# MystenLabs/dapol

Measured on AMD Instinct MI355X. Metric: entities/sec (tree build + 64-bit range-proof gen), 2^20 leaves, 1/2/4/8 GPU, higher is better.
Workload: dtype int32 limbs (255-bit modular integers)

## Files before the change

### dapol_amd/csrc/host_range.inc

```

#include <cstdlib>
#include "policy_plan.inc"
#include "prove_plan.inc"

struct MsmTiming {
    std::vector<hipEvent_t> ev;
    std::vector<int> kind;
    size_t used = 0;
    bool enabled = false;
    size_t kernels[2] = {0, 0};
    ~MsmTiming() { for (auto e : ev) (void)hipEventDestroy(e); }
    hipError_t mark(hipStream_t st, int k = 0) {
        if (!enabled) return hipSuccess;
        if (used == ev.size()) {
            hipEvent_t e;
            hipError_t r = hipEventCreate(&e);
            if (r != hipSuccess) return r;
            ev.push_back(e);
        }
        if ((used & 1) == 0) { if (kind.size() <= used / 2) kind.push_back(k); else kind[used / 2] = k; }
        return hipEventRecord(ev[used++], st);
    }
    void count(int k, size_t n) { if (enabled) kernels[k] += n; }
    double total_ms(int k) {
// ... 192 lines not shown
}

static int32_t queue_chunk(dapol_ctx* ctx, const ProvePlan& P, const ProveLane& L, RangeArgs A, hipStream_t st, ForkGuard& fg, uint32_t* d_err,
                           MsmTiming* tm) {
    const size_t cb = A.B;
    const int fs_shape = P.fs_shape, nf_rounds = P.nf_rounds();
    sc* const stab_buf = A.stab;
    if (!P.stab_main) A.stab = nullptr;
    const unsigned g_wave = (unsigned)cb, g_lane = nblk(cb, 64), g_dig = (unsigned)(cb * (size_t)(A.TP / 64));
    const unsigned g_gsdig = nblk(cb * (size_t)(2 * A.N), 64);
    hipLaunchKernelGGL(k_rp_nonce_key, dim3(g_lane), dim3(64), 0, st, A); LAUNCH_CHECK();
    if (P.gs) hipLaunchKernelGGL(k_rp_nonces_gs, dim3(g_gsdig), dim3(64), 0, st, A);
    else hipLaunchKernelGGL(k_rp_nonces, dim3(g_dig), dim3(64), 0, st, A);
    LAUNCH_CHECK();
    if (P.side_A) {
        HIPCHK(hipEventRecord(ctx->ev_fork, st));
        HIPCHK(hipStreamWaitEvent(ctx->side[2], ctx->ev_fork, 0));
        fg.forked(2);
        hipLaunchKernelGGL(k_rp_A, dim3(g_wave), dim3(64), 0, ctx->side[2], A, ctx->tv); LAUNCH_CHECK();
        HIPCHK(hipEventRecord(ctx->ev_join[2], ctx->side[2]));
        FAULT_AFTER_FORK("prove_A");
    } else if (P.a_lane(cb)) {
        hipLaunchKernelGGL(k_rp_A_lane, dim3(g_lane), dim3(64), 0, st, A, ctx->tv); LAUNCH_CHECK();
    } else {
        hipLaunchKernelGGL(k_rp_A, dim3(g_wave), dim3(64), 0, st, A, ctx->tv); LAUNCH_CHECK();
    }
    if (tm) HIPCHK(tm->mark(st));
    launch_main_msm(ctx, P, L, A, st, -1, tm); LAUNCH_CHECK();
    if (tm) HIPCHK(tm->mark(st));
    if (P.side_A) { HIPCHK(hipStreamWaitEvent(st, ctx->ev_join[2], 0)); fg.joined(2); }
    LAUNCH_FS(k_rp_finish1, fs_shape, cb, st, A, ctx->tv); LAUNCH_CHECK();
    hipLaunchKernelGGL(k_rp_poly, dim3(g_wave * (unsigned)A.fs_parts), dim3(64), 0, st, A); LAUNCH_CHECK();
    LAUNCH_FS(k_rp_finish2, fs_shape, cb, st, A, ctx->tv); LAUNCH_CHECK();
    hipLaunchKernelGGL(k_rp_lr, dim3(g_wave * (unsigned)A.fs_parts), dim3(64), 0, st, A); LAUNCH_CHECK();
    if (fs_shape == 2) hipLaunchKernelGGL(k_rp_finish3<2>, dim3(g_wave), dim3(64), 0, st, A);
    else hipLaunchKernelGGL(k_rp_finish3<0>, dim3(g_lane), dim3(64), 0, st, A);
    LAUNCH_CHECK();
    for (int k = 0; k < nf_rounds; k++) {
        if (P.gs) hipLaunchKernelGGL(k_rp_round_prep_gs, dim3(g_gsdig), dim3(64), 0, st, A, k);
        else hipLaunchKernelGGL(k_rp_round_prep, dim3(g_dig), dim3(64), 0, st, A, k);
        LAUNCH_CHECK();
        hipLaunchKernelGGL(k_rp_round_ip, dim3(g_wave), dim3(64), 0, st, A, k); LAUNCH_CHECK();
        if (tm) HIPCHK(tm->mark(st));
        launch_main_msm(ctx, P, L, A, st, k, tm); LAUNCH_CHECK();
        if (tm) HIPCHK(tm->mark(st));
        LAUNCH_FS(k_rp_round_finish, fs_shape, cb, st, A, ctx->tv, k); LAUNCH_CHECK();
        hipLaunchKernelGGL(k_rp_fold, dim3(fold_blocks(A, cb, k)), dim3(256), 0, st, A, k);
        LAUNCH_CHECK();
    }
    if (nf_rounds == A.lgN) {
        hipLaunchKernelGGL(k_rp_final, dim3(g_lane), dim3(64), 0, st, A, d_err); LAUNCH_CHECK();
        return DAPOL_OK;
    }
    if (P.gs_mat) hipLaunchKernelGGL(k_rp_mat_prep_gs, dim3(g_gsdig), dim3(64), 0, st, A);
    else hipLaunchKernelGGL(k_rp_mat_prep, dim3(g_dig), dim3(64), 0, st, A);
    LAUNCH_CHECK();
    if (tm) HIPCHK(tm->mark(st, 1));
    { int32_t rc = launch_materialise(ctx, P, L, A, st, tm); if (rc) return rc; }
    if (tm) HIPCHK(tm->mark(st, 1));
    const unsigned g_tail = (unsigned)(cb * (size_t)(P.tail_n / 32));
    {
        RangeArgs Ai = A;
        Ai.stab = P.stab_tail ? stab_buf : nullptr;
        if (P.tail_rpl == 4) hipLaunchKernelGGL(k_rp_tail_table4, dim3(nblk(cb * (size_t)(2 * P.tail_n / 4), 64)), dim3(64), 0, st, Ai);
        else hipLaunchKernelGGL(k_rp_tail_table, dim3(g_tail), dim3(64), 0, st, Ai);
        LAUNCH_CHECK();
    }
    RangeArgs At = A;
    At.N = P.tail_n; At.lgN = P.tail_lgn; At.TP = 2 * P.tail_n; At.wbits = TAIL_WBITS; At.nwin = TAIL_NWIN; At.nsplit = 0;
    At.a = A.tail_a; At.b = A.tail_b; At.s1 = A.tail_s1; At.s2 = A.tail_s2;
    At.stab = P.stab_tail ? stab_buf : nullptr;
    At.out_round0 = nf_rounds;
    const TableView tvt{A.tailT, 1, TAIL_WBITS, 0, 0};
    for (int k = 0; k < P.tail_lgn; k++) {
        hipLaunchKernelGGL(k_rp_round_prep, dim3(g_tail), dim3(64), 0, st, At, k); LAUNCH_CHECK();
        hipLaunchKernelGGL(k_rp_round_ip, dim3(g_wave), dim3(64), 0, st, At, k); LAUNCH_CHECK();
        if (P.tail_gs) {
            hipLaunchKernelGGL(k_rp_tail_gs, dim3(nblk(2 * cb, TAIL_GS_LISTS)), dim3(TAIL_GS_BLOCK), 0, st, At, tvt, k, L.gsacc); LAUNCH_CHECK();
            hipLaunchKernelGGL(k_rp_tail_combine, dim3(nblk(2 * cb, 64)), dim3(64), 0, st, At, L.gsacc);
        } else launch_msm_tail(st, At, tvt, k, P.tail_lpl);
        LAUNCH_CHECK();
        LAUNCH_FS(k_rp_round_finish, fs_shape, cb, st, At, ctx->tv, k); LAUNCH_CHECK();
        hipLaunchKernelGGL(k_rp_fold, dim3(fold_blocks(At, cb, k)), dim3(256), 0, st, At, k);
        LAUNCH_CHECK();
    }
    hipLaunchKernelGGL(k_rp_final, dim3(g_lane), dim3(64), 0, st, At, d_err); LAUNCH_CHECK();
    return DAPOL_OK;
}

static int32_t range_prove_device(dapol_ctx* ctx, int n, int m, size_t B, const uint64_t* d_vals, const uint32_t* d_blind,
                                  const uint32_t* d_Vc, const uint32_t* d_seed, const uint64_t* d_stream, uint64_t slot_base,
                                  const uint32_t* d_tape, uint32_t* d_out, MsmTiming* tm, size_t tape_stride = 0, uint32_t sub_k = 1,
                                  size_t out_stride = 0, PendingProve* pend = nullptr) {
    ProveShape s{};
    s.n = n; s.m = m; s.B = B;
    s.tail_length = ctx->opt.tail_length; s.small_call_max = ctx->opt.small_call_max; s.generator_stationary = ctx->opt.generator_stationary;
    s.streams = ctx->opt.streams; s.gs_tile_rows = ctx->opt.gs_tile_rows; s.gs_slices = ctx->opt.gs_slices; s.chunk_proofs = ctx->opt.chunk_proofs;
    s.wbits = ctx->tv.wbits; s.nwin = ctx->tv.nwin_c(); s.hi_split = ctx->tv.hi_split;
    s.n_cu = ctx->n_cu; s.resident_waves = ctx->resident_waves();
    s.budget_bytes = scratch_budget_bytes(ctx);
    s.timed = tm != nullptr;
    ProvePlan P = plan_range_prove(s);
    for (bool lowered = false;; lowered = true) {
        hipError_t e = ctx->scratch.ensure(P.lane_bytes() * P.nlanes);
        if (e == hipSuccess) {
            if (lowered) P.finalise(s, P.chunk, P.nlanes);
            break;
        }
        (void)hipGetLastError();
        if (e != hipErrorOutOfMemory || (P.nlanes == 1 && P.chunk <= 64)) return fail_hip(e, "scratch allocation", __FILE__, __LINE__);
        if (P.nlanes > 1) P.nlanes--;
        else P.chunk = (P.chunk + 1) / 2;
    }
    const size_t chunk = P.chunk, slots = (size_t)m * (2 * (size_t)n + 4);
    const int nlanes = P.nlanes;
    RangeArgs A{};
    A.n = n; A.m = m; A.N = P.N; A.lgN = P.lgN; A.TP = P.TP;
    A.out_words = 72 + 16 * A.lgN;
    A.seed = d_seed; A.slot_base = slot_base;
    A.wbits = s.wbits; A.nwin = s.nwin;
    A.tail_n = P.tail_n; A.use_hi = P.use_hi ? 1 : 0; A.fs_parts = P.fs_parts; A.mat_round = P.nf_rounds();
    A.stream_id = d_stream;
    A.tape_stride = (uint32_t)(tape_stride ? tape_stride : slots);
    A.tape = d_tape;
    A.sub_k = sub_k ? sub_k : 1; A.sub_slots = (uint32_t)slots;
    A.out = d_out; A.out_stride = out_stride ? out_stride : (size_t)A.out_words;
    ProveLane lanes[4];
    hipStream_t lane_stream[4] = {ctx->stream, ctx->side[0], ctx->side[1], ctx->side[2]};
    for (int ln = 0; ln < nlanes; ln++) lanes[ln] = carve_lane(P, A, (uint8_t*)ctx->scratch.p + P.lane_bytes() * ln);
    DevBuf<uint32_t> err_own;
    DevBuf<uint32_t>& err = pend ? pend->err : err_own;
    HIPCHK(err.alloc(1));
    HIPCHK(hipMemsetAsync(err.p, 0, 4, ctx->stream));
    ForkGuard fg(ctx);
    if (nlanes > 1) {
        HIPCHK(hipEventRecord(ctx->ev_fork, ctx->stream));
        for (int ln = 1; ln < nlanes; ln++) { HIPCHK(hipStreamWaitEvent(lane_stream[ln], ctx->ev_fork, 0)); fg.forked(ln - 1); }
    }
    size_t chunk_no = 0;
    for (size_t first = 0; first < B; first += chunk, chunk_no++) {
        const int ln = (int)(chunk_no % (size_t)nlanes);
        if (chunk_no == 2) FAULT_AFTER_FORK("prove_lanes");
        RangeArgs Ac = lanes[ln].A;
        Ac.B = B - first < chunk ? B - first : chunk;
        Ac.vals = d_vals + first * m;
        Ac.blind = d_blind + first * m * 8;
        Ac.Vc = d_Vc + first * m * 8;
        Ac.p0 = first;
        int32_t rc = queue_chunk(ctx, P, lanes[ln], Ac, lane_stream[ln], fg, err.p, tm);
        if (rc) return rc;
    }
    for (int ln = 1; ln < nlanes; ln++) {
        HIPCHK(hipEventRecord(ctx->ev_join[ln - 1], lane_stream[ln]));
        HIPCHK(hipStreamWaitEvent(ctx->stream, ctx->ev_join[ln - 1], 0));
        fg.joined(ln - 1);
    }
    if (pend) {
        pend->ctx = ctx;
        pend->h_err_p = ctx->h_pinned + pend->pinned_slot;
        HIPCHK(hipMemcpyAsync(pend->h_err_p, err.p, 4, hipMemcpyDeviceToHost, ctx->stream));
        pend->armed = true;
        return DAPOL_OK;
    }
    uint32_t h_err = 0;
    HIPCHK(hipMemcpyAsync(&h_err, err.p, 4, hipMemcpyDeviceToHost, ctx->stream));
    HIPCHK(hipStreamSynchronize(ctx->stream));
    if (h_err) return fail(DAPOL_ERR_INVALID_ARGUMENT, "prover drew a zero challenge (ProofError::MaliciousDealer)");
    return DAPOL_OK;
}

struct EventPair {
    hipEvent_t a = nullptr, b = nullptr;
    ~EventPair() { if (a) (void)hipEventDestroy(a); if (b) (void)hipEventDestroy(b); }
// ... 43 lines not shown
```

### dapol_amd/csrc/kernels_range.h

```cpp
#pragma once
#include <hip/hip_runtime.h>
#include <type_traits>
#include "kernels_ctx_tree.h"
#include "ge_quad.h"

namespace dapol {

struct ProofState {
    uint64_t strobe[25];
    uint32_t pos, pos_begin;
    uint32_t err, pad_;
    sc y, z, y_inv, x, w, u, u_inv;
    sc a_bl, s_bl, t1, t2, t1_bl, t2_bl, t_x, cL, cR;
    uint32_t nkey[8];
};

struct RangeArgs {
    int n, m, N, lgN, TP;
    int wbits, nwin;
    size_t B;
    const uint64_t* vals;
    const uint32_t* blind;
    const uint32_t* Vc;
    const uint32_t* seed;
    const uint64_t* stream_id;
    uint64_t slot_base;
    const uint32_t* tape;
    uint32_t tape_stride;
    uint32_t sub_k, sub_slots;
    size_t p0;
    sc* a; sc* b; sc* s1; sc* s2;
    sc* stab;
    dig_t* dig;
    int nsplit;
    int use_hi;
    int fs_parts;
    sc* fs_part;
    ProofState* st;
    int32_t* PA; int32_t* P0; int32_t* P1;
    int mat_round;
    int tail_n;
    int32_t* tailT;
    sc* tail_a; sc* tail_b; sc* tail_s1; sc* tail_s2;
    uint32_t* out;
    size_t out_stride;
    int out_words;
    int out_round0;
};

#ifndef DAPOL_TAIL_WBITS
#define DAPOL_TAIL_WBITS 5
#endif
enum { TAIL_WBITS = DAPOL_TAIL_WBITS, TAIL_NWIN = 253 / TAIL_WBITS + 1, TAIL_ENTRIES = (1 << (TAIL_WBITS - 1)) + 1, TAIL_ROW_WORDS = TAIL_ENTRIES * 32 };
enum { MSM_PLAIN = 0, MSM_MATERIALIZE = 1, MSM_TAIL = 2 };
enum { STAB_ROUNDS = 6, STAB_N = 1 << STAB_ROUNDS };

__device__ __forceinline__ void proof_row(const RangeArgs& A, size_t b, size_t& e, uint32_t& j) {
    const size_t g = A.p0 + b;
    if (A.sub_k <= 1) { e = g; j = 0; }
    else { e = g / A.sub_k; j = (uint32_t)(g - e * A.sub_k); }
}
__device__ __forceinline__ uint32_t* proof_out(const RangeArgs& A, size_t b) {
    size_t e; uint32_t j;
    proof_row(A, b, e, j);
    return A.out + e * A.out_stride + (size_t)j * (size_t)A.out_words;
}
__device__ __forceinline__ void tape_wide(uint32_t* w16, const RangeArgs& A, size_t b, uint32_t slot) {
    size_t e; uint32_t j;
    proof_row(A, b, e, j);
    const uint32_t first = j * A.sub_slots;
    if (A.tape) {
        const uint4* p = reinterpret_cast<const uint4*>(A.tape + (e * (size_t)A.tape_stride + first + slot) * 16);
        for (int i = 0; i < 4; i++) { uint4 q = p[i]; w16[4 * i] = q.x; w16[4 * i + 1] = q.y; w16[4 * i + 2] = q.z; w16[4 * i + 3] = q.w; }
    } else {
        uint32_t key[8];
        for (int i = 0; i < 8; i++) key[i] = A.st[b].nkey[i];
        seed_wide(w16, key, 2u, A.stream_id[e], A.slot_base + first + slot);
    }
}
__global__ __launch_bounds__(64) void k_rp_nonce_key(RangeArgs A) {
    size_t b = (size_t)blockIdx.x * 64 + threadIdx.x;
    if (b >= A.B || A.tape) return;
    uint32_t key[8], w[16];
    for (int i = 0; i < 8; i++) key[i] = A.seed[i];
    size_t e; uint32_t sj;
    proof_row(A, b, e, sj);
    seed_wide(w, key, 6u, A.stream_id[e], A.slot_base + (uint64_t)sj * A.sub_slots);
    for (int i = 0; i < 8; i++) key[i] = w[i];
    seed_wide(w, key, 7u, (uint64_t)A.n, (uint64_t)A.m);
    for (int i = 0; i < 8; i++) key[i] = w[i];
    for (int j0 = 0; j0 < A.m; j0 += 31) {
        const int n_ent = 1 + ((A.m - j0 < 31) ? A.m - j0 : 31);
        const int n_blk = (n_ent + 1) / 2;
        uint32_t cv[8], blk[16], o[16];
        blake3_iv(cv);
        for (int i = 0; i < n_blk; i++) {
            for (int h = 0; h < 2; h++) {
                const int e = 2 * i + h;
                if (e == 0) { for (int k = 0; k < 8; k++) blk[k] = key[k]; }
                else if (e < n_ent) ld8(blk + 8 * h, A.Vc + (b * A.m + j0 + e - 1) * 8);
                else { for (int k = 0; k < 8; k++) blk[8 + k] = 0; }
            }
            const bool last = i == n_blk - 1;
            blake3_compress(o, cv, blk, 0, (last && (n_ent & 1)) ? 32u : 64u, (i == 0 ? B3_CHUNK_START : 0u) | (last ? (B3_CHUNK_END | B3_ROOT) : 0u));
            for (int k = 0; k < 8; k++) cv[k] = o[k];
        }
        for (int k = 0; k < 8; k++) key[k] = cv[k];
    }
// ... 332 lines not shown
    size_t g = (size_t)blockIdx.x * 64 + threadIdx.x;
    if (g >= n_gen) return;
    const int32_t* src = PS + g * (size_t)nsplit * 40;
    ge_p3 acc, p, r;
    ld_p3(acc, src);
    for (int s = 1; s < nsplit; s++) {
        ld_p3(p, src + (size_t)s * 40);
        ge_add(r, acc, p);
        acc = r;
    }
    st_p3(tailT + g * TAIL_ROW_WORDS, acc);
}

template <int ENTRIES>
__device__ __forceinline__ void build_niels_row(int32_t* row) {
    ge_p3 base, mul;
    ld_p3(base, row);
    mul = base;
    fe pre[ENTRIES - 1];
#pragma unroll
    for (int e = 1; e < ENTRIES; e++) {
        if (e > 1) { ge_p3 t; ge_add(t, mul, base); mul = t; }
        int32_t* slot = row + e * 32;
        for (int i = 0; i < FE_NL; i++) { slot[i] = mul.X.v[i]; slot[FE_NL + i] = mul.Y.v[i]; slot[2 * FE_NL + i] = mul.Z.v[i]; }
        if (e == 1) pre[0] = mul.Z;
        else fe_mul(pre[e - 1], pre[e - 2], mul.Z);
    }
    fe inv;
    fe_invert(inv, pre[ENTRIES - 2]);
#pragma unroll
    for (int e = ENTRIES - 1; e >= 1; e--) {
        int32_t* slot = row + e * 32;
        fe X, Y, Z, zi, x, y;
        for (int i = 0; i < FE_NL; i++) { X.v[i] = slot[i]; Y.v[i] = slot[FE_NL + i]; Z.v[i] = slot[2 * FE_NL + i]; }
        if (e > 1) { fe_mul(zi, inv, pre[e - 2]); fe t; fe_mul(t, inv, Z); inv = t; }
        else zi = inv;
        fe_mul(x, X, zi);
        fe_mul(y, Y, zi);
        ge_niels q;
        ge_to_niels(q, x, y);
        niels_store_entry(slot, q);
    }
    ge_niels id;
    ge_niels_identity(id);
    niels_store_entry(row, id);
}

__device__ __forceinline__ void tail_row_vectors(const RangeArgs& A, size_t b, int g) {
    const int T = A.tail_n;
    sc one, v;
    sc_zero(one); one.v[0] = 1;
    int i = g < T ? g : g - T;
    if (g == 0) stab_init(A, b);
    st_sc((g < T ? A.tail_s1 : A.tail_s2) + b * T + i, one);
    ld_sc(v, (g < T ? A.a : A.b) + b * A.N + i);
    st_sc((g < T ? A.tail_a : A.tail_b) + b * T + i, v);
}
__global__ __launch_bounds__(64) void k_rp_tail_table(RangeArgs A) {
    const int T = A.tail_n, bpp = (2 * T) >> 6;
    size_t b = blockIdx.x / bpp;
    int g = (int)(blockIdx.x % bpp) * 64 + threadIdx.x;
    build_niels_row<TAIL_ENTRIES>(A.tailT + (b * (size_t)(2 * T) + g) * TAIL_ROW_WORDS);
    tail_row_vectors(A, b, g);
}

template <int ENTRIES>
__device__ __forceinline__ void niels_row_multiples(int32_t* row, fe& total) {
    ge_p3 base, mul;
    ld_p3(base, row);
    mul = base;
#pragma nounroll
    for (int e = 1; e < ENTRIES; e++) {
        if (e > 1) { ge_p3 t; ge_add(t, mul, base); mul = t; }
        int32_t* slot = row + e * 32;
        for (int i = 0; i < FE_NL; i++) { slot[i] = mul.X.v[i]; slot[FE_NL + i] = mul.Y.v[i]; slot[2 * FE_NL + i] = mul.Z.v[i]; }
        if (e == 1) total = mul.Z;
        else { fe t; fe_mul(t, total, mul.Z); total = t; }
    }
}
template <int ENTRIES>
__device__ __forceinline__ void niels_row_finish(int32_t* row, fe inv) {
    fe pre[ENTRIES - 1];
#pragma unroll
    for (int e = 1; e < ENTRIES; e++) {
        const int32_t* slot = row + e * 32;
        fe Z;
        for (int i = 0; i < FE_NL; i++) Z.v[i] = slot[2 * FE_NL + i];
        if (e == 1) pre[0] = Z;
        else fe_mul(pre[e - 1], pre[e - 2], Z);
    }
#pragma unroll
    for (int e = ENTRIES - 1; e >= 1; e--) {
        int32_t* slot = row + e * 32;
        fe X, Y, Z, zi, x, y;
        for (int i = 0; i < FE_NL; i++) { X.v[i] = slot[i]; Y.v[i] = slot[FE_NL + i]; Z.v[i] = slot[2 * FE_NL + i]; }
        if (e > 1) { fe_mul(zi, inv, pre[e - 2]); fe t; fe_mul(t, inv, Z); inv = t; }
        else zi = inv;
        fe_mul(x, X, zi);
        fe_mul(y, Y, zi);
        ge_niels q;
        ge_to_niels(q, x, y);
        niels_store_entry(slot, q);
    }
    ge_niels id;
    ge_niels_identity(id);
    niels_store_entry(row, id);
// ... 584 lines not shown
```

### dapol_amd/csrc/kernels_range_gs.h

```cpp
#pragma once
#include "kernels_range.h"

namespace dapol {

__device__ __forceinline__ void write_digits_gs(const RangeArgs& A, size_t p, int sp, const uint32_t* c) {
    const size_t L = A.B * (size_t)A.nwin;
    int32_t* out = reinterpret_cast<int32_t*>(A.dig) + ((((size_t)(sp >> 2)) * L + p) << 2) + (sp & 3);
    const size_t wstride = A.B * (size_t)4;
    const int W = A.wbits, NW = A.nwin, half = 1 << (W - 1);
    const uint32_t mask = (1u << W) - 1;
    uint32_t x[8];
#pragma unroll
    for (int i = 0; i < 8; i++) x[i] = c[i];
    int carry = 0;
#pragma nounroll
    for (int w = 0; w < NW; w++) {
        const int b = (int)(x[0] & mask) + carry;
        carry = (b >= half && w != NW - 1) ? 1 : 0;
        out[(size_t)w * wstride] = b - (carry << W);
#pragma unroll
        for (int i = 0; i < 7; i++) x[i] = (x[i] >> W) | (x[i + 1] << (32 - W));
        x[7] >>= W;
    }
}

#define GS_BLOCKS(A, vb) for (size_t vb = blockIdx.x, nb_ = ((size_t)(A).B * (size_t)(2 * (A).N) + 63) / 64; vb < nb_; vb += gridDim.x)
__device__ __forceinline__ bool gs_thread(const RangeArgs& A, size_t vblock, size_t& p, int& sp) {
    const size_t t = vblock * 64 + threadIdx.x;
    const size_t quad = t >> 2, sp4 = quad / A.B;
    p = quad - sp4 * A.B;
    sp = (int)(4 * sp4) + (int)(t & 3);
    return sp4 < (size_t)(2 * A.N) / 4;
}

__global__ __launch_bounds__(64) void k_rp_nonces_gs(RangeArgs A) {
    GS_BLOCKS(A, vb) {
        size_t p;
        int sp;
        if (!gs_thread(A, vb, p, sp)) continue;
        const int side = sp >= A.N ? 1 : 0, q = sp - side * A.N;
        const int j = q / A.n, ii = q - j * A.n;
        const uint32_t slot = (uint32_t)(j * (2 * A.n + 2) + 2 + ii + (side ? A.n : 0));
        sc s;
        tape_scalar(s, A, p, slot);
        st_sc((side ? A.s2 : A.s1) + p * A.N + q, s);
        uint32_t c[8];
        sc_from_mont(c, s);
        write_digits_gs(A, p, sp, c);
    }
}

__global__ __launch_bounds__(64) void k_rp_round_prep_gs(RangeArgs A, int round) {
    GS_BLOCKS(A, vb) {
        size_t p;
        int sp;
        if (!gs_thread(A, vb, p, sp)) continue;
        const int side = sp >= A.N ? 1 : 0, q = sp - side * A.N;
        const int lgh = A.lgN - 1 - round, half = 1 << lgh;
        bool isH;
        const int j = term_generator(round, A.N, A.lgN, side, q, isH);
        const int off = j & (half - 1);
        const bool upper = (j >> lgh) & 1;
// ... 107 lines not shown
        load(o, s);
        ge_add(r, acc, o);
        acc = r;
    }
    for (int i = 0; i < FE_NL; i++) {
        ap[(size_t)i * Ltot] = acc.X.v[i]; ap[(size_t)(FE_NL + i) * Ltot] = acc.Y.v[i];
        ap[(size_t)(2 * FE_NL + i) * Ltot] = acc.Z.v[i]; ap[(size_t)(3 * FE_NL + i) * Ltot] = acc.T.v[i];
    }
}

__global__ __launch_bounds__(64) void k_rp_gs_combine(RangeArgs A, const int32_t* __restrict__ accs, size_t side_words, int nslice, int LW) {
    const size_t Ltot = A.B * (size_t)LW * (size_t)nslice;
    const size_t t = (size_t)blockIdx.x * 64 + threadIdx.x;
    if (t >= 2 * A.B) return;
    const int side = t >= A.B ? 1 : 0;
    const size_t p = t - (size_t)side * A.B;
    accs += (size_t)side * side_words;
    auto load = [&](ge_p3& r, int w) {
        const int32_t* ap = accs + (size_t)w * A.B + p;
        for (int i = 0; i < FE_NL; i++) {
            r.X.v[i] = ap[(size_t)i * Ltot]; r.Y.v[i] = ap[(size_t)(FE_NL + i) * Ltot];
            r.Z.v[i] = ap[(size_t)(2 * FE_NL + i) * Ltot]; r.T.v[i] = ap[(size_t)(3 * FE_NL + i) * Ltot];
        }
    };
    ge_p3 acc, t2, r;
    load(acc, LW - 1);
#pragma nounroll
    for (int w = LW - 2; w >= 0; w--) {
#pragma nounroll
        for (int d = 0; d < A.wbits; d++) ge_dbl(acc, acc, d == A.wbits - 1);
        load(t2, w);
        ge_add(r, acc, t2);
        acc = r;
    }
    st_p3((side ? A.P1 : A.P0) + p * 40, acc);
}

enum { MAT_GROUP = 16 };
enum { GS_ACC_SLOTS = 32, GS_MAX_SLICES = 16, GS_FULL_LANES = 3072 * 64 };
static_assert(GS_ACC_SLOTS >= MAT_GROUP && GS_ACC_SLOTS >= 2 * GS_MAX_SLICES, "accumulator slots");

__global__ __launch_bounds__(64) void k_rp_mat_prep_gs(RangeArgs A) {
    GS_BLOCKS(A, vb) {
        size_t p;
        int sp;
        if (!gs_thread(A, vb, p, sp)) continue;
        const int side = sp >= A.N ? 1 : 0, rem = sp - side * A.N;
        const int per = A.N / A.tail_n, cls = rem / per, k = rem - cls * per;
        sc s;
        coeff_plain(s, A, p, A.mat_round, cls + k * A.tail_n, side != 0);
        write_digits_gs(A, p, sp, s.v);
    }
}

__global__ __launch_bounds__(64, DAPOL_GS_OCC) void k_rp_mat_gs(RangeArgs A, TableView tbl, int side, int cls, int hi, int LW, int32_t* __restrict__ accs) {
    const size_t LM = A.B * (size_t)LW, L = A.B * (size_t)A.nwin;
    const size_t lane = (size_t)blockIdx.x * 64 + threadIdx.x;
    if (lane >= LM) return;
    cls += (int)blockIdx.y;
    accs += (size_t)blockIdx.y * 4 * FE_NL * LM;
    const int w = (int)(lane / A.B);
    const size_t p = lane - (size_t)w * A.B;
    const int wd = w + (hi ? LW : 0);
    if (wd >= A.nwin) return;
    ge_p3 acc;
    int32_t* ap = accs + lane;
    if (!hi) ge_identity(acc);
    else {
#pragma unroll
        for (int i = 0; i < FE_NL; i++) {
            acc.X.v[i] = ap[(size_t)i * LM]; acc.Y.v[i] = ap[(size_t)(FE_NL + i) * LM];
            acc.Z.v[i] = ap[(size_t)(2 * FE_NL + i) * LM]; acc.T.v[i] = ap[(size_t)(3 * FE_NL + i) * LM];
        }
    }
    const int per = A.N / A.tail_n;
    const dapol_v4i* dg = reinterpret_cast<const dapol_v4i*>(A.dig) + ((size_t)(side * A.N + cls * per) >> 2) * L + (size_t)wd * A.B + p;
    dapol_v4i d4 = dg[0], dn = d4;
#pragma nounroll
    for (int k = 0; k < per; k++) {
        if ((k & 3) == 0 && k + 4 < per) dn = dg[(size_t)((k >> 2) + 1) * L];
        const int d = d4.x;
        d4.x = d4.y; d4.y = d4.z; d4.z = d4.w;
        if ((k & 3) == 3) d4 = dn;
        const int row = gen_row(tbl, A.n, cls + k * A.tail_n, side != 0);
        tbl_madd(acc, tbl, hi ? tbl.row_hi(row) : row, d);
    }
#pragma unroll
    for (int i = 0; i < FE_NL; i++) {
        ap[(size_t)i * LM] = acc.X.v[i]; ap[(size_t)(FE_NL + i) * LM] = acc.Y.v[i];
        ap[(size_t)(2 * FE_NL + i) * LM] = acc.Z.v[i]; ap[(size_t)(3 * FE_NL + i) * LM] = acc.T.v[i];
    }
}

__global__ __launch_bounds__(64) void k_rp_mat_gs_horner(RangeArgs A, int side, int cls0, int ncls, int LW, const int32_t* __restrict__ accs) {
    const size_t LM = A.B * (size_t)LW;
    const size_t t = (size_t)blockIdx.x * 64 + threadIdx.x;
    if (t >= (size_t)ncls * A.B) return;
    const int c = (int)(t / A.B);
    const size_t p = t - (size_t)c * A.B;
    const int32_t* slot = accs + (size_t)c * 4 * FE_NL * LM;
    auto load = [&](ge_p3& r, int w) {
        const int32_t* ap = slot + (size_t)w * A.B + p;
        for (int i = 0; i < FE_NL; i++) {
            r.X.v[i] = ap[(size_t)i * LM]; r.Y.v[i] = ap[(size_t)(FE_NL + i) * LM];
            r.Z.v[i] = ap[(size_t)(2 * FE_NL + i) * LM]; r.T.v[i] = ap[(size_t)(3 * FE_NL + i) * LM];
        }
    };
    ge_p3 acc, q, r;
    load(acc, LW - 1);
#pragma nounroll
    for (int w = LW - 2; w >= 0; w--) {
#pragma nounroll
        for (int d = 0; d < A.wbits; d++) ge_dbl(acc, acc, d == A.wbits - 1);
        load(q, w);
        ge_add(r, acc, q);
        acc = r;
    }
    const int T = A.tail_n;
    st_p3(A.tailT + (p * (size_t)(2 * T) + (size_t)(side * T + cls0 + c)) * TAIL_ROW_WORDS, acc);
}

enum { TAIL_GS_BLOCK = 256, TAIL_GS_LISTS = TAIL_GS_BLOCK / TAIL_NWIN, TAIL_REC_WORDS = 4 * FE_NL };
static_assert(TAIL_GS_LISTS >= 1, "a list's windows fit a block");
__global__ __launch_bounds__(TAIL_GS_BLOCK, DAPOL_GS_OCC) void k_rp_tail_gs(RangeArgs A, TableView tbl, int round, int32_t* __restrict__ recs) {
    const int li = (int)threadIdx.x / TAIL_NWIN, w = (int)threadIdx.x - li * TAIL_NWIN;
    const size_t list = (size_t)blockIdx.x * TAIL_GS_LISTS + li;
    if (li >= TAIL_GS_LISTS || list >= 2 * A.B) return;
    const size_t p = list >> 1;
    const int side = (int)(list & 1);
// ... 37 lines not shown
```

### dapol_amd/csrc/prove_plan.inc

```
#pragma once
#include <cstddef>
#include <cstdint>
#include <cstdlib>

enum { FS_PARTS_MAX = 8 };
enum { TAIL_RPL_DEFAULT = 4 };
enum { TAIL_GS_DEFAULT = 1 };

struct ProveShape {
    int n, m;
    size_t B;
    int tail_length, small_call_max, generator_stationary, streams, gs_tile_rows, gs_slices;
    long long chunk_proofs;
    int wbits, nwin, hi_split;
    int n_cu;
    size_t resident_waves;
    size_t budget_bytes;
    bool timed;
};

struct ProvePlan {
    int N, lgN, TP;
    int nwin, hi_split;
    int tail_n, tail_lgn;
    bool small_call, use_hi;
    int fs_shape, fs_parts;
    bool gs, gs_mat;
    int gs_LW, acc_slots;
    bool stab_main, stab_tail;
    int msm_split, mat_split, quad_split;
    size_t dig_elems, stab_bytes, acc_bytes, per_proof, split_bytes;
    size_t chunk;
    int nlanes;
    bool big_batch;
    int lpl, tail_lpl;
    bool side_A;
    bool tail_gs;
    int tail_order;
    size_t tail_rec_bytes;
    int tail_rpl, tail_rpl_forced;
    int gs_tile, gs_slices_forced, mat_cpl_forced;
    bool gs_tile_set, a_lane_ok;
    const char* lpl_env;

    int part_split() const { return quad_split ? quad_split : msm_split; }
    int nf_rounds() const { return lgN - tail_lgn; }
    size_t lane_bytes() const { return (chunk * per_proof + 8192 + split_bytes + 4095) / 4096 * 4096; }

    int slices_for(size_t cb) const {
        if (gs_slices_forced) return gs_slices_forced <= acc_slots / 2 ? gs_slices_forced : acc_slots / 2;
        int ns = cb <= 4096 ? 16 : (cb < 40000 ? 8 : (cb < 65536 ? 4 : 1));
        if (N < 1024) {
            const size_t lanes = cb * (size_t)gs_LW;
            ns = lanes >= 2 * (size_t)GS_FULL_LANES ? 1 : (lanes >= (size_t)GS_FULL_LANES ? 2 : (lanes >= (size_t)GS_FULL_LANES / 2 ? 4 : (lanes >= (size_t)GS_FULL_LANES / 8 ? 8 : 16)));
        }
        while (ns > 1 && ((N / ns) % 4 != 0 || N / ns < 32)) ns /= 2;
        return ns;
    }
    int tile_for(size_t cb, int ns) const {
        int tile = (!gs_tile_set && cb * (size_t)nwin < 2 * (size_t)GS_FULL_LANES && N / ns >= 32) ? 32 : gs_tile;
        if (gs_LW < nwin && !gs_tile_set) tile = tile / 2;
        return tile;
    }
    int mat_LW() const { return hi_split ? hi_split : nwin; }
    int mat_cpl(size_t cb) const {
        if (mat_cpl_forced) return mat_cpl_forced;
        int cpl = 1;
        while (cpl < MAT_GROUP && cb * (size_t)mat_LW() * (size_t)cpl < GS_FULL_LANES) cpl *= 2;
        return cpl;
    }
    bool a_lane(size_t cb) const { return !side_A && gs && N < 1024 && cb >= 4096 && a_lane_ok; }

    void finalise(const ProveShape& s, size_t chunk_, int nlanes_);
};

static int small_split_cap(bool use_hi) {
    if (const char* e = knob("DAPOL_SMALL_SPLIT")) { int v = atoi(e); if (v >= 1 && v <= 64 && !(v & (v - 1))) return v; }
    return use_hi ? 64 : 8;
}
static size_t quad_max_waves(size_t dflt) {
    if (const char* e = knob("DAPOL_QUAD_MAX_WAVES")) { long long v = atoll(e); if (v > 0) return (size_t)v; }
    return dflt;
}
static int pick_lanes_per_list(size_t proofs, int terms_per_list, int nwin, int wbits, const int* cand, int ncand, size_t resident, size_t n_simd,
                               bool shared_simd = false) {
    int best = cand[0];
    double best_cost = 1e300;
    const size_t occ = n_simd ? (resident + n_simd - 1) / n_simd : 1;
    for (int i = 0; i < ncand; i++) {
        int lpl = cand[i];
        size_t waves = (proofs + (size_t)(32 / lpl) - 1) / (size_t)(32 / lpl);
        const size_t full = waves / resident, rem = waves % resident;
        const size_t krem = rem ? (rem + n_simd - 1) / (n_simd ? n_simd : 1) : 0;
// ... 61 lines not shown
    P.tail_n = tail_n; P.tail_lgn = tail_lgn;
    const size_t T = (size_t)tail_n;
    size_t dig_elems = (size_t)s.nwin * P.TP;
    if (dig_elems < (size_t)TAIL_NWIN * 2 * T) dig_elems = (size_t)TAIL_NWIN * 2 * T;
    P.dig_elems = dig_elems;
    const bool no_stab = knob("DAPOL_NO_STAB") != nullptr;
    P.stab_main = !no_stab && (tail_n ? lgN - tail_lgn : lgN - 1) <= STAB_ROUNDS;
    P.stab_tail = !no_stab && tail_n && tail_lgn - 1 <= STAB_ROUNDS;
    bool gs_possible = (!small_call && N % 4 == 0 && N >= 1024 && B >= gs_min) || gs_small;
    if (s.generator_stationary) gs_possible = s.generator_stationary > 0 && !small_call && N % 4 == 0 && N >= 64;
    if (gs_env >= 0) gs_possible = gs_env != 0 && !small_call && N % 4 == 0 && N >= 64;
    int acc_slots = GS_ACC_SLOTS;
    if (N < 1024) {
        acc_slots = 2 * (N / 32 < GS_MAX_SLICES ? N / 32 : GS_MAX_SLICES);
        if (tail_n && acc_slots < MAT_GROUP) acc_slots = MAT_GROUP;
    }
    P.acc_slots = acc_slots;
    P.acc_bytes = gs_possible ? (size_t)acc_slots * s.nwin * 4 * FE_NL * 4 : 0;
    P.stab_bytes = (P.stab_main || P.stab_tail) ? (size_t)2 * 2 * STAB_N * sizeof(sc) : 0;
    if (const char* e = knob("DAPOL_TAIL_ORDER")) P.tail_order = (e[0] == 'g' && e[1] == 's' && !e[2]) ? 1 : ((e[0] == 'p' && e[1] == 's' && !e[2]) ? -1 : 0);
    if (const char* e = knob("DAPOL_TAIL_ROWS_PER_LANE")) { int v = atoi(e); if (v == 1 || v == 4) P.tail_rpl_forced = v; }
    P.tail_rec_bytes = (P.tail_order > 0 && tail_n && P.acc_bytes < tail_rec_need()) ? tail_rec_need() - P.acc_bytes : 0;
    P.per_proof = 4 * (size_t)N * sizeof(sc) + dig_elems * sizeof(dig_t) + (sizeof(ProofState) + 15) / 16 * 16 + 3 * 160 +
                  2 * T * TAIL_ROW_WORDS * 4 + 4 * T * sizeof(sc) + FS_PARTS_MAX * 3 * sizeof(sc) + P.stab_bytes + P.acc_bytes + P.tail_rec_bytes;
    int nlanes = s.streams > 0 ? s.streams : 1;
    if (const char* e = knob("DAPOL_STREAMS")) { int v = atoi(e); if (v >= 1 && v <= 4) nlanes = v; }
    size_t chunk = s.budget_bytes / nlanes / P.per_proof;
    if (chunk < 1) chunk = 1;
    if (chunk > B) chunk = B;
    {
        const char* const e_chunk = knob("DAPOL_CHUNK");
        const bool chunk_set = e_chunk || s.chunk_proofs > 0;
        const long long chunk_forced = e_chunk ? atoll(e_chunk) : s.chunk_proofs;
        const size_t rw = s.resident_waves;
        size_t ppw = 16;
        if (e_lpl) { int v = atoi(e_lpl); if (v == 2 || v == 4 || v == 8) ppw = (size_t)(32 / v); }
        const size_t big_chunk = (3 * rw * ppw <= chunk) ? 3 * rw * ppw : ((2 * rw * ppw <= chunk) ? 2 * rw * ppw : rw * ppw), std_chunk = 5 * rw * 4;
        P.big_batch = !chunk_set && N >= 1024 && B >= big_chunk && chunk >= big_chunk;
        size_t cap = chunk_set ? (size_t)chunk_forced : (P.big_batch ? big_chunk : std_chunk);
        const size_t small_unit = rw * 64 / (size_t)(s.hi_split ? s.hi_split : s.nwin);
        if (gs_small && !chunk_set) cap = 8 * small_unit;
        if (cap < 64) cap = 64;
        if (chunk > cap) chunk = cap;
        if (gs_small && !chunk_set && chunk > small_unit) chunk -= chunk % small_unit;
    }
    while (nlanes > 1 && chunk * (size_t)(nlanes - 1) >= B) nlanes--;
    P.chunk = chunk; P.nlanes = nlanes;
    bool gs = P.big_batch || (!small_call && B >= gs_min && chunk >= 1024 && N >= 1024 && N % 4 == 0) || (gs_small && chunk >= 64);
    if (s.generator_stationary) gs = s.generator_stationary > 0 && !small_call && N % 4 == 0 && N >= 64;
    if (gs_env >= 0) gs = gs_env != 0 && !small_call && N % 4 == 0 && N >= 64;
    if (!gs_possible) gs = false;
    P.gs = gs;
    P.gs_mat = gs && tail_n && (N / tail_n) % 4 == 0 && !knob("DAPOL_NO_GS_MAT");
    P.gs_tile = s.gs_tile_rows > 0 ? s.gs_tile_rows : 16;
    const char* const e_tile = knob("DAPOL_GS_TILE");
    P.gs_tile_set = s.gs_tile_rows > 0 || e_tile;
    if (e_tile) { int v = atoi(e_tile); if (v >= 4 && v % 4 == 0) P.gs_tile = v; }
    P.gs_slices_forced = (s.gs_slices > 0 && N % (4 * s.gs_slices) == 0 && N / s.gs_slices >= 4) ? s.gs_slices : 0;
    if (const char* e = knob("DAPOL_GS_SLICES")) { int v = atoi(e); if ((v == 1 || v == 2 || v == 4 || v == 8 || v == 16) && N % (4 * v) == 0 && N / v >= 4) P.gs_slices_forced = v; }
    P.gs_LW = (gs && N < 1024 && s.hi_split && !knob("DAPOL_NO_GS_HI")) ? s.hi_split : s.nwin;
    if (const char* e = knob("DAPOL_GS_MAT_CPL")) { int v = atoi(e); if (v >= 1 && v <= MAT_GROUP) P.mat_cpl_forced = v; }
    P.a_lane_ok = !knob("DAPOL_NO_A_LANE");
    P.msm_split = 1; P.mat_split = 1;
    if (small_call) {
        const int cap = small_split_cap(use_hi), min_terms = use_hi ? 1 : 4;
        while (P.msm_split < cap && (size_t)P.msm_split * 2 * B <= 2048 && N / 32 / (P.msm_split * 2) >= min_terms) P.msm_split *= 2;
        if (tail_n && !knob("DAPOL_NO_SPLIT_MAT"))
            while (P.mat_split < 8 && (size_t)(P.mat_split * 2) * B * (size_t)(tail_n / 32) <= 4096 && N / tail_n / (P.mat_split * 2) >= 2) P.mat_split *= 2;
    }
    P.fs_parts = 1;
    if (small_call && B <= 64 && !knob("DAPOL_NO_FS_PARTS")) {
        const int iters = (N + 63) / 64;
        while (P.fs_parts < FS_PARTS_MAX && iters / (P.fs_parts * 2) >= 2) P.fs_parts *= 2;
    }
    if (use_hi && P.msm_split > 1 && (size_t)P.msm_split * 4 * B <= quad_max_waves(2048) && N % (8 * P.msm_split * 4) == 0 && !knob("DAPOL_NO_QUAD")) P.quad_split = P.msm_split * 4;
    P.split_bytes = (P.part_split() > 1 ? (2 * chunk * (size_t)P.part_split() * 160 + 255) / 256 * 256 : 0) +
                    (P.mat_split > 1 ? (chunk * 2 * T * (size_t)P.mat_split * 160 + 255) / 256 * 256 : 0);
    P.finalise(s, chunk, nlanes);
    return P;
}

void ProvePlan::finalise(const ProveShape& s, size_t chunk_, int nlanes_) {
    chunk = chunk_; nlanes = nlanes_;
    const char* const e_tail_lpl = knob("DAPOL_TAIL_LPL");
    lpl = msm_lanes_per_list(N, big_batch, lpl_env);
    tail_lpl = tail_lanes_per_list(small_call, e_tail_lpl);
    if (small_call) lpl = 32;
    else if (!lpl_env && N >= 1024 && !big_batch && chunk < 32768) {
        const int cand[2] = {8, 16};
        lpl = pick_lanes_per_list(chunk, N, s.nwin, s.wbits, cand, 2, s.resident_waves, (size_t)s.n_cu * 4);
    }
    if (!e_tail_lpl && !small_call && tail_n && chunk < 65536) {
        const int cand[4] = {2, 4, 8, 32};
        tail_lpl = pick_lanes_per_list(chunk, tail_n, TAIL_NWIN, TAIL_WBITS, cand, 4, s.resident_waves, (size_t)s.n_cu * 4, true);
    }
    tail_gs = tail_n != 0 && (tail_order > 0 || (tail_order == 0 && TAIL_GS_DEFAULT && gs && !small_call && N >= 1024 && chunk >= 65536 && acc_bytes >= tail_rec_need()));
    tail_rpl = tail_rpl_forced ? tail_rpl_forced : ((TAIL_RPL_DEFAULT == 4 && gs && !small_call && N >= 1024 && chunk >= 65536) ? 4 : 1);
    if (!tail_n || (2 * tail_n) % 4 != 0) tail_rpl = 1;
    side_A = small_call && nlanes == 1 && s.B <= 64 && !s.timed && !knob("DAPOL_NO_SIDE_A");
}
```

### dapol_amd/csrc/sc.h

```cpp
#pragma once
#include "consts.h"

namespace dapol {

struct sc {
    uint32_t v[8];
};

DAPOL_HD void sc_zero(sc& r) {
    for (int i = 0; i < 8; i++) r.v[i] = 0;
}
DAPOL_HD void sc_one_mont(sc& r) {
    for (int i = 0; i < 8; i++) r.v[i] = SC_R1[i];
}
DAPOL_HD bool sc_is_zero(const sc& a) {
    uint32_t o = 0;
    for (int i = 0; i < 8; i++) o |= a.v[i];
    return o == 0;
}

DAPOL_HD uint32_t sc_addc(uint32_t a, uint32_t b, uint32_t cin, uint32_t& cout) {
#if defined(__clang__) && !defined(DAPOL_SC_NO_BUILTIN_CARRY)
    return __builtin_addc(a, b, cin, &cout);
#else
// ... 225 lines not shown
        w[8] = (uint32_t)(((int32_t)((uint32_t)acc << 16)) >> 16);
    }
    if (f[8] < 0) {
        uint32_t c = 1;
        for (int i = 0; i < 9; i++) w[i] = sc_addc(~w[i], 0u, c, c);
    }
    for (int k = 0; k < 4 && (w[8] >> 31); k++) {
        uint32_t c = 0;
        for (int i = 0; i < 9; i++) w[i] = sc_addc(w[i], i < 8 ? SC_L[i] : 0u, c, c);
    }
    for (int k = 0; k < 4; k++) {
        uint32_t t9[9], bw = 0;
        for (int i = 0; i < 9; i++) t9[i] = sc_subb(w[i], i < 8 ? SC_L[i] : 0u, bw, bw);
        if (t9[8] >> 31) break;
        for (int i = 0; i < 9; i++) w[i] = t9[i];
    }
    sc x, k3;
    for (int i = 0; i < 8; i++) { x.v[i] = w[i]; k3.v[i] = SC_R3[i]; }
    sc_montmul(out, x, k3);
}

DAPOL_HD void sc_pow_mont(sc& r, const sc& a, uint32_t e) {
    sc acc, base = a;
    sc_one_mont(acc);
    while (e) {
        if (e & 1) sc_montmul(acc, acc, base);
        sc_montsq(base, base);
        e >>= 1;
    }
    r = acc;
}

DAPOL_HD void sc_recode_s8(int16_t* d, const uint32_t* x) {
    int carry = 0;
    for (int i = 0; i < 32; i++) {
        int b = (int)((x[i >> 2] >> (8 * (i & 3))) & 0xff) + carry;
        carry = (b > 127 && i < 31) ? 1 : 0;
        d[i] = (int16_t)(b - (carry << 8));
    }
}

template <typename F>
DAPOL_HD void sc_recode_w(int W, int NW, const uint32_t* x, F out) {
    int carry = 0;
    for (int i = 0; i < NW; i++) {
        int o = i * W, wd = o >> 5, sh = o & 31;
        uint32_t lo = wd < 8 ? x[wd] >> sh : 0u;
        uint32_t hi = (sh && wd + 1 < 8) ? (x[wd + 1] << (32 - sh)) : 0u;
        int b = (int)((lo | hi) & ((1u << W) - 1)) + carry;
        carry = (b >= (1 << (W - 1)) && i < NW - 1) ? 1 : 0;
        out(i, b - (carry << W));
    }
}

}
```

Baseline: 57240.

## Share materialise digit prep across classes and add compile-time signed-window recode

Adds two prep optimisations that are on by default. The first is a fully unrolled signed-digit recoder specialised for the 17x15 and 16x16 window geometries, used in the generator-stationary digit writer. The second is a shared materialisation prep path. When the stab table is in use, it computes digits for only one class per side and indexes them from every class, and it loads tail_s2 from s2 instead of writing ones. This is meant to cut redundant scalar coefficient computation and digit writes in the materialise prep stage. The price is a dependence on the stab table having already absorbed the class-specific factors, so the change is correctness-sensitive.

```diff
diff --git a/dapol_amd/csrc/host_range.inc b/dapol_amd/csrc/host_range.inc
--- a/dapol_amd/csrc/host_range.inc
+++ b/dapol_amd/csrc/host_range.inc
@@ -268,7 +268,8 @@
         hipLaunchKernelGGL(k_rp_final, dim3(g_lane), dim3(64), 0, st, A, d_err); LAUNCH_CHECK();
         return DAPOL_OK;
     }
-    if (P.gs_mat) hipLaunchKernelGGL(k_rp_mat_prep_gs, dim3(g_gsdig), dim3(64), 0, st, A);
+    if (P.prep_share) hipLaunchKernelGGL(k_rp_mat_prep_gs_shared, dim3(nblk(cb * (size_t)(2 * (A.N / A.tail_n)), 64)), dim3(64), 0, st, A);
+    else if (P.gs_mat) hipLaunchKernelGGL(k_rp_mat_prep_gs, dim3(g_gsdig), dim3(64), 0, st, A);
     else hipLaunchKernelGGL(k_rp_mat_prep, dim3(g_dig), dim3(64), 0, st, A);
     LAUNCH_CHECK();
     if (tm) HIPCHK(tm->mark(st, 1));
@@ -335,6 +336,7 @@
     A.out_words = 72 + 16 * A.lgN;
     A.seed = d_seed; A.slot_base = slot_base;
     A.wbits = s.wbits; A.nwin = s.nwin;
+    A.prep = (P.prep_recode ? PREP_RECODE : 0) | (P.prep_share ? PREP_SHARE : 0);
     A.tail_n = P.tail_n; A.use_hi = P.use_hi ? 1 : 0; A.fs_parts = P.fs_parts; A.mat_round = P.nf_rounds();
     A.stream_id = d_stream;
     A.tape_stride = (uint32_t)(tape_stride ? tape_stride : slots);
diff --git a/dapol_amd/csrc/kernels_range.h b/dapol_amd/csrc/kernels_range.h
--- a/dapol_amd/csrc/kernels_range.h
+++ b/dapol_amd/csrc/kernels_range.h
@@ -18,6 +18,7 @@
 struct RangeArgs {
     int n, m, N, lgN, TP;
     int wbits, nwin;
+    int prep;
     size_t B;
     const uint64_t* vals;
     const uint32_t* blind;
@@ -54,6 +55,7 @@
 enum { TAIL_WBITS = DAPOL_TAIL_WBITS, TAIL_NWIN = 253 / TAIL_WBITS + 1, TAIL_ENTRIES = (1 << (TAIL_WBITS - 1)) + 1, TAIL_ROW_WORDS = TAIL_ENTRIES * 32 };
 enum { MSM_PLAIN = 0, MSM_MATERIALIZE = 1, MSM_TAIL = 2 };
 enum { STAB_ROUNDS = 6, STAB_N = 1 << STAB_ROUNDS };
+enum { PREP_RECODE = 1, PREP_SHARE = 2 };
 
 __device__ __forceinline__ void proof_row(const RangeArgs& A, size_t b, size_t& e, uint32_t& j) {
     const size_t g = A.p0 + b;
@@ -492,6 +494,7 @@
     sc_zero(one); one.v[0] = 1;
     int i = g < T ? g : g - T;
     if (g == 0) stab_init(A, b);
+    if (g >= T && (A.prep & PREP_SHARE)) ld_sc(one, A.s2 + b * A.N + i);
     st_sc((g < T ? A.tail_s1 : A.tail_s2) + b * T + i, one);
     ld_sc(v, (g < T ? A.a : A.b) + b * A.N + i);
     st_sc((g < T ? A.tail_a : A.tail_b) + b * T + i, v);
diff --git a/dapol_amd/csrc/kernels_range_gs.h b/dapol_amd/csrc/kernels_range_gs.h
--- a/dapol_amd/csrc/kernels_range_gs.h
+++ b/dapol_amd/csrc/kernels_range_gs.h
@@ -8,6 +8,10 @@
     int32_t* out = reinterpret_cast<int32_t*>(A.dig) + ((((size_t)(sp >> 2)) * L + p) << 2) + (sp & 3);
     const size_t wstride = A.B * (size_t)4;
     const int W = A.wbits, NW = A.nwin, half = 1 << (W - 1);
+    if (A.prep & PREP_RECODE) {
+        if (W == 17 && NW == 15) { sc_recode_fixed<17, 15>(c, [&](int w, int digit) { out[(size_t)w * wstride] = digit; }); return; }
+        if (W == 16 && NW == 16) { sc_recode_fixed<16, 16>(c, [&](int w, int digit) { out[(size_t)w * wstride] = digit; }); return; }
+    }
     const uint32_t mask = (1u << W) - 1;
     uint32_t x[8];
 #pragma unroll
@@ -221,6 +225,17 @@
         write_digits_gs(A, p, sp, s.v);
     }
 }
+__global__ __launch_bounds__(64) void k_rp_mat_prep_gs_shared(RangeArgs A) {
+    const int per = A.N / A.tail_n;
+    const size_t t = (size_t)blockIdx.x * 64 + threadIdx.x;
+    const size_t quad = t >> 2, sp4 = quad / A.B, p = quad - sp4 * A.B;
+    if (sp4 >= (size_t)(2 * per) / 4) return;
+    const int sp = (int)(4 * sp4) + (int)(t & 3);
+    const int side = sp >= per ? 1 : 0, k = sp - side * per;
+    sc s;
+    coeff_plain(s, A, p, A.mat_round, k * A.tail_n, side != 0);
+    write_digits_gs(A, p, sp, s.v);
+}
 
 __global__ __launch_bounds__(64, DAPOL_GS_OCC) void k_rp_mat_gs(RangeArgs A, TableView tbl, int side, int cls, int hi, int LW, int32_t* __restrict__ accs) {
     const size_t LM = A.B * (size_t)LW, L = A.B * (size_t)A.nwin;
@@ -243,7 +258,7 @@
         }
     }
     const int per = A.N / A.tail_n;
-    const dapol_v4i* dg = reinterpret_cast<const dapol_v4i*>(A.dig) + ((size_t)(side * A.N + cls * per) >> 2) * L + (size_t)wd * A.B + p;
+    const dapol_v4i* dg = reinterpret_cast<const dapol_v4i*>(A.dig) + ((size_t)((A.prep & PREP_SHARE) ? side * per : side * A.N + cls * per) >> 2) * L + (size_t)wd * A.B + p;
     dapol_v4i d4 = dg[0], dn = d4;
 #pragma nounroll
     for (int k = 0; k < per; k++) {
diff --git a/dapol_amd/csrc/prove_plan.inc b/dapol_amd/csrc/prove_plan.inc
--- a/dapol_amd/csrc/prove_plan.inc
+++ b/dapol_amd/csrc/prove_plan.inc
@@ -6,6 +6,9 @@
 enum { FS_PARTS_MAX = 8 };
 enum { TAIL_RPL_DEFAULT = 4 };
 enum { TAIL_GS_DEFAULT = 1 };
+#ifndef DAPOL_PREP_V2_PARTS
+#define DAPOL_PREP_V2_PARTS 3
+#endif
 
 struct ProveShape {
     int n, m;
@@ -39,6 +42,7 @@
     int tail_order;
     size_t tail_rec_bytes;
     int tail_rpl, tail_rpl_forced;
+    bool prep_recode, prep_share;
     int gs_tile, gs_slices_forced, mat_cpl_forced;
     bool gs_tile_set, a_lane_ok;
     const char* lpl_env;
@@ -206,6 +210,12 @@
     if (!gs_possible) gs = false;
     P.gs = gs;
     P.gs_mat = gs && tail_n && (N / tail_n) % 4 == 0 && !knob("DAPOL_NO_GS_MAT");
+    {
+        const char* const e = knob("DAPOL_PREP");
+        const int parts = (e && e[0] == 'v' && e[1] == '1' && !e[2]) ? 0 : DAPOL_PREP_V2_PARTS;
+        P.prep_recode = gs && (parts & 1);
+        P.prep_share = P.gs_mat && P.stab_main && (parts & 2);
+    }
     P.gs_tile = s.gs_tile_rows > 0 ? s.gs_tile_rows : 16;
     const char* const e_tile = knob("DAPOL_GS_TILE");
     P.gs_tile_set = s.gs_tile_rows > 0 || e_tile;
diff --git a/dapol_amd/csrc/sc.h b/dapol_amd/csrc/sc.h
--- a/dapol_amd/csrc/sc.h
+++ b/dapol_amd/csrc/sc.h
@@ -301,5 +301,19 @@
         out(i, b - (carry << W));
     }
 }
-
-}
+template <int W, int NW, typename F>
+DAPOL_HD void sc_recode_fixed(const uint32_t* x, F out) {
+    static_assert(W >= 2 && W <= 31 && NW >= 1 && W * (NW - 1) < 256, "window geometry");
+    int carry = 0;
+#pragma unroll
+    for (int i = 0; i < NW; i++) {
+        const int o = i * W, wd = o >> 5, sh = o & 31;
+        uint32_t v = x[wd] >> sh;
+        if (sh + W > 32 && wd + 1 < 8) v |= x[wd + 1] << (32 - sh);
+        const int b = (int)(v & ((1u << W) - 1)) + carry;
+        carry = (i < NW - 1 && b >= (1 << (W - 1))) ? 1 : 0;
+        out(i, b - (carry << W));
+    }
+}
+
+}
```

After: 57860, median of 6. 1.01x the previous value.
